# lxd99/TPNet

Hardware: AMD Instinct MI355X
Metric: temporal edges/sec (proj-update + pairwise readout) (higher is better)
Workload: dtype f32; 1 GPU; C2: Wikipedia-shape d=128 B=1000, L=3, synthetic S(8227,1000,E,span) stream of 2399000 edges, decoder-level unit (2 readouts + update per edge); batch=1000, dim=128, num_layer=3, nodes=9228, parallelism=single GPU

## Files before the change

tpnet_amd/csrc/plan.hip:

```cpp
#include "wplan_common.hpp"
#include "arena.hpp"
#include "sort_tmp.hpp"

#include <cstdlib>
#include <cstring>
#include <rocprim/block/block_radix_sort.hpp>
#include <rocprim/device/device_radix_sort.hpp>
#include <rocprim/device/device_segmented_radix_sort.hpp>
#include <rocprim/iterator/counting_iterator.hpp>
#include <rocprim/iterator/transform_iterator.hpp>

#ifdef TPNET_STAMPS
#define PSTAMP(slot)                                                                          \
    do {                                                                                      \
        if (dbg && blockIdx.x == 0 && threadIdx.x == 0) {                                     \
            dbg[(slot) * 2 + 0] = __builtin_amdgcn_s_memtime();                               \
            dbg[(slot) * 2 + 1] = __builtin_amdgcn_s_memrealtime();                           \
        }                                                                                     \
    } while (0)
#else
#define PSTAMP(slot) do { } while (0)
#endif

namespace tpnet {
// ... 606 lines not shown
    while (K < Kmax && (int64_t)K * K < (int64_t)num * nb) ++K;
    const int64_t nw0 = (nb + K - 1) / K;
    return (int)((nb + nw0 - 1) / nw0);
}

WPlanner choose_wplanner(const tpnet_state& st, const WPlan* p, int64_t Ec, int64_t batch, int K, uint32_t flags) {
    static const int no3 = TPNET_DEV_INT(NO_PLAN3, 0);
    static const int max3 = TPNET_DEV_INT(PLAN3_MAX_BATCHES, 1 << 30);
    const bool small = batch <= PLAN_ONE_MAX;
    if (!(flags & (TPNET_FLAG_PLAN_SORTED | TPNET_FLAG_PLAN_HASHED)) &&
        (p ? wplan_dense_applies(st, *p, Ec, batch, K) : small && wplan_dense_eligible(st.N, st.d, st.L, batch)))
        return {wplan_dense_build, wplan_dense_writeback, true, 256};
    if (!(flags & TPNET_FLAG_PLAN_SORTED) &&
        (p ? !no3 && (Ec + batch - 1) / batch <= max3 && wplan3_applies(st, Ec, batch, K) : small))
        return {wplan3_build, wplan3_writeback, true, WIN_MAX_WINDOWS};
    return {wplan_build, launch_wwriteback, false, 0};
}

bool wplan_medium_chains(int d) {
    static const int off = TPNET_DEV_INT(NO_MEDIUM, 0);
    if (off || d % 4 != 0) return false;
    const Geom g = pick_geom(d);
    return g.w == 4 && d == g.lpp * g.vpl * 4;
}

uint32_t wplan_heavy_threshold(int K, int64_t batch, int d) {
    static const int env = TPNET_DEV_INT(WIN_HEAVY, 0);
    if (env > 0) return (uint32_t)env;
    if (wplan_medium_chains(d)) return 128u;
    const int64_t t = (int64_t)K * batch * d / 24576;
    return (uint32_t)(t < 16 ? 16 : (t > 96 ? 96 : t));
}

int64_t wplan_max_chunk_edges(int64_t batch, int d, int L) {
    static const char* env = TPNET_DEV_STR(WIN_CHUNK_MB);
    const int64_t log_cap = (env ? (int64_t)atoi(env) : 16384) << 20;
    int64_t e = log_cap / (2 * (int64_t)L * d * 4);
    const int64_t hard = (int64_t)(WREF_SLOT_MASK >> 1);
    if (e > hard) e = hard;
    if (e > 65535 * batch) e = 65535 * batch;
    e = e / batch * batch;
    return e < batch ? batch : e;
}

static void wplan_layout(Arena& a, WPlan& p, int64_t Ec, int64_t batch, int64_t N, int d, int L, bool own_log) {
    const size_t nc = 2 * (size_t)Ec;
    const size_t nw = (size_t)((Ec + batch - 1) / batch);
    plan_layout(a, p.base, Ec, batch);
    a.skip(256);
    p.wscr = a.take<uint32_t>(3 * align256(nc * 4) / 4);
    a.skip(nc * 2);
    p.wdesc = a.take<WinDesc>(nw);
    a.skip(256);
    p.e_ref = a.take<uint32_t>(3 * (size_t)Ec);
    p.e_g = a.take<float>(3 * (size_t)Ec);
    p.log = own_log ? a.take<float>(nc * (size_t)L * (size_t)d) : nullptr;
    p.node_lo = a.take<uint32_t>((size_t)N);
    p.node_hi = a.take<uint32_t>((size_t)N);
    p.inv = a.take<uint32_t>(nc);
    p.rhead = a.take<uint32_t>(nc);
    const size_t zero0 = a.off;
    p.wmask = a.take<unsigned long long>((size_t)N);
    p.wcls = a.take<uint32_t>(2 * WIN_MAX_WINDOWS * 8 + WIN_MAX_WINDOWS);
    p.wzero_bytes = a.off - zero0;
    p.wtab = a.take<char>(wplan3_table_bytes(Ec, batch));
    p.wblk = (uint32_t*)a.take<char>(wplan3_blk_bytes(Ec, batch));
// ... 245 lines not shown
            const uint32_t c8 = ch.cnt > 255u ? 255u : ch.cnt;
            lk[j] = chain_head ? (((uint32_t)w << 8) | (255u - c8)) : lk_none;
            if (chain_head) p.chains_sparse[j] = ch;
        }
    }
}

__global__ void k_gather_chains(WPlan p, const uint32_t* __restrict__ lk, const uint32_t* __restrict__ lv, int64_t nc,
                                int64_t nw, uint32_t heavy_threshold, uint32_t lk_none) {
    if (blockIdx.x == gridDim.x - 1) {
        auto lb = [&](uint32_t key) {
            int64_t lo = 0, hi = nc;
            while (lo < hi) {
                const int64_t mid = (lo + hi) >> 1;
                if (lk[mid] < key) lo = mid + 1; else hi = mid;
            }
            return lo;
        };
        const uint32_t thr8 = heavy_threshold > 254u ? 254u : heavy_threshold;
        for (int64_t w = threadIdx.x; w < nw; w += blockDim.x) {
            const int64_t a = lb((uint32_t)w << 8);
            const int64_t h = lb(((uint32_t)w << 8) | (255u - thr8));
            const int64_t z = lb((uint32_t)(w + 1) << 8);
            WinDesc D;
            D.start = (uint32_t)a;
            D.n_heavy = (uint32_t)(h - a);
            D.n_chains = (uint32_t)(z - a);
            D.n_ext = D.n_heavy;
            D.n_ext1 = D.n_heavy;
            {
                const int64_t m = lb(((uint32_t)w << 8) | (255u - (WIN_MED_MIN - 1u)));
                D.n_med = (uint32_t)((m > h ? m : h) - a);
            }
            D.pad1 = D.pad2 = 0;
            p.wdesc[w] = D;
        }
        return;
    }
    for (int64_t i = (int64_t)blockIdx.x * blockDim.x + threadIdx.x; i < nc; i += (int64_t)(gridDim.x - 1) * blockDim.x) {
        if (lk[i] >= lk_none) continue;
        p.chains[i] = p.chains_sparse[lv[i]];
    }
}

template <typename K>
__device__ __forceinline__ void edge_refs(uint32_t bx, uint32_t nbx, WPlan p, const K* __restrict__ keys, const int64_t* __restrict__ src,
                            const int64_t* __restrict__ dst, const int64_t* __restrict__ neg, int64_t Ec, int64_t B,
                            int64_t N, int batch_bits, double lambda, const NodeMeta* __restrict__ meta) {
    const int nwhich = neg ? 3 : 2;
    const int64_t tot = (int64_t)nwhich * Ec;
    const int64_t nc = 2 * Ec;
    for (int64_t x = (int64_t)bx * blockDim.x + threadIdx.x; x < tot; x += (int64_t)nbx * blockDim.x) {
        const int which = (int)(x / Ec);
        const int64_t e = x - (int64_t)which * Ec;
        int64_t node = which == 0 ? src[e] : (which == 1 ? dst[e] : neg[e]);
        if ((uint64_t)node >= (uint64_t)N) node = 0;
        const int64_t b = e / B;
        uint32_t ref;
        float g;
        bool done = false;
        if (which < 2) {
            const int64_t e0b = b * B;
            const int64_t neb = (Ec - e0b < B) ? (Ec - e0b) : B;
            const uint32_t orig = (uint32_t)(2 * e0b + (which ? neb : 0) + (e - e0b));
            done = version_before_own_run<K>(p, keys, batch_bits, node, b, p.inv[orig], p.base.desc, meta, lambda,
                                             p.base.desc[b].now, ref, g);
        }
// ... 82 lines not shown
```

tpnet_amd/csrc/tpnet_common.h:

```cpp
#pragma once
#include <hip/hip_runtime.h>
#include <stdint.h>
#include <stdlib.h>
#include <initializer_list>
#include <new>
#include "../../include/tpnet_hip.h"
#include "tpnet_dev.h"
#include "event_set.hpp"

#ifdef TPNET_DEV
static inline int tpnet_dev_env_int(const char* name, int dflt) { const char* v = getenv(name); return v ? atoi(v) : dflt; }
#define TPNET_DEV_INT(NAME, DFLT) tpnet_dev_env_int("TPNET_DEV_" #NAME, (DFLT))
#define TPNET_DEV_STR(NAME) getenv("TPNET_DEV_" #NAME)
#else
#define TPNET_DEV_INT(NAME, DFLT) (DFLT)
#define TPNET_DEV_STR(NAME) ((const char*)nullptr)
#endif

namespace tpnet {

struct NodeMeta {
    uint32_t ver;
    uint32_t pad0;
    double tref[2];
// ... 203 lines not shown
               int64_t Ec, int64_t batch, double now_time, const double* t_prev_dev, double lambda, uint32_t flags,
               hipStream_t s);

static constexpr uint32_t ROLE_READOUT = 1u << 16;
static constexpr uint32_t ROLE_UPDATE = 1u << 17;
static constexpr uint32_t STEP_FUSE = 1u << 18;
static constexpr uint32_t STEP_ITEMS_FIRST = 1u << 20;
static constexpr uint32_t STEP_HAS_POS = 1u << 21;
static constexpr uint32_t STEP_HAS_NEG = 1u << 22;
static constexpr uint32_t PLAN_FUSE = 1u << 19;

static constexpr int WIN_MAX_BATCHES = 64;
static constexpr uint32_t WREF_TABLE = 1u << 31;
static constexpr uint32_t WREF_RUN_HEAD = 1u << 30;
static constexpr uint32_t WREF_RUN_TAIL = 1u << 29;
static constexpr uint32_t WREF_BLK_HEAD = 1u << 28;
static constexpr uint32_t WREF_BLK_TAIL = 1u << 27;
static constexpr uint32_t WREF_LAST_RUN = 1u << 26;
static constexpr uint32_t WREF_SLOT_MASK = (1u << 26) - 1;
static constexpr int WIN_MAX_WINDOWS = 64;
static constexpr int WIN_BLOCK = 8;

static constexpr uint32_t WIN_MED_MIN = 16;
__host__ __device__ inline int wchain_med_classes(uint32_t thr) {
    const int c = (32 - __builtin_clz(thr | 1u)) - 4;
    return c < 0 ? 0 : (c > 6 ? 6 : c);
}
__host__ __device__ inline int wchain_class(uint32_t cnt, uint32_t thr) {
    if (cnt > thr) return 0;
    const int dl = (32 - __builtin_clz(thr | 1u)) - (32 - __builtin_clz(cnt | 1u));
    return 1 + (dl > 6 ? 6 : (dl < 0 ? 0 : dl));
}

struct WinDesc {
    uint32_t start;
    uint32_t n_heavy;
    uint32_t n_chains;
    uint32_t n_ext;
    uint32_t n_ext1;
    uint32_t n_med;
    uint32_t pad1, pad2;
};

struct Chain {
    uint32_t j0;
    uint32_t cnt;
    int32_t target;
    uint32_t prev_ref;
    float g_first;
    uint32_t pad0, pad1, pad2;
};
static_assert(sizeof(Chain) == 32, "Chain must be 32 bytes");

struct WRec {
    int32_t partner;
    float coef;
    uint32_t ref;
    float g;
    float dec;
    int32_t target;
    uint32_t bc;
    uint32_t spare;
};
static_assert(sizeof(WRec) == 32, "WRec must be 32 bytes");

struct WPlan {
    Plan base;
    WRec* rec;
    uint32_t* wscr;
    WinDesc* wdesc;
    Chain* chains;
    Chain* chains_sparse;
    uint32_t* lk_in;
    uint32_t* lk_out;
    uint32_t* lv_in;
// ... 28 lines not shown
    const int64_t *src, *dst, *neg;
    const double* t;
    int64_t Ec, batch;
    double now_time;
    const double* t_prev_dev;
    double lambda;
    bool want_readout;
    bool replay;
    int64_t own = -1;
    uint32_t* status = nullptr;
};
int wplan_build(const tpnet_state& st, const WPlan& p, const WPlanArgs& a, hipStream_t s);
int wplan3_build(const tpnet_state& st, const WPlan& p, const WPlanArgs& a, hipStream_t s);
int wplan_dense_build(const tpnet_state& st, const WPlan& p, const WPlanArgs& a, hipStream_t s);
int launch_wwriteback(const tpnet_state& st, const WPlan& p, int64_t Ec, int64_t batch, uint32_t launch_id, hipStream_t s, int64_t own = -1);
int wplan3_writeback(const tpnet_state& st, const WPlan& p, int64_t Ec, int64_t batch, uint32_t launch_id, hipStream_t s, int64_t own = -1);
int wplan_dense_writeback(const tpnet_state& st, const WPlan& p, int64_t Ec, int64_t batch, uint32_t launch_id, hipStream_t s, int64_t own = -1);
bool wplan3_applies(const tpnet_state& st, int64_t Ec, int64_t batch, int K);
size_t wplan3_table_bytes(int64_t Ec, int64_t batch);
size_t wplan3_blk_bytes(int64_t Ec, int64_t batch);
bool wplan_dense_eligible(int64_t N, int d, int L, int64_t batch);
size_t wplan_dense_bytes(int64_t Ec, int64_t batch, int64_t N, int d, int L);
bool wplan_dense_applies(const tpnet_state& st, const WPlan& p, int64_t Ec, int64_t batch, int K);
bool wplan_dense_applies_shard(const tpnet_state& st, const WPlan& p, int64_t Ec, int64_t batch, int K);

struct WPlanner {
    decltype(&wplan_build) build;
    decltype(&launch_wwriteback) writeback;
    bool replayable;
    int max_windows;
};
WPlanner choose_wplanner(const tpnet_state& st, const WPlan* p, int64_t Ec, int64_t batch, int K, uint32_t flags);
uint32_t wplan_heavy_threshold(int K, int64_t batch, int d);
bool wplan_medium_chains(int d);
int launch_wstep(const tpnet_state& st, const StreamArgs& a, const WPlan& p, int64_t j, int64_t Ec, int64_t batch,
                 double lambda, uint32_t flags, hipStream_t s);
int check_state(const tpnet_state* st);

static inline bool aligned16(std::initializer_list<const void*> ps) {
    uintptr_t a = 0;
    for (const void* p : ps) a |= reinterpret_cast<uintptr_t>(p);
    return (a & 15) == 0;
}

extern thread_local int g_last_hip_error;
#define TPNET_HIP_TRY(expr)                                   \
    do {                                                      \
        hipError_t _e = (expr);                               \
        if (_e != hipSuccess) {                               \
            tpnet::g_last_hip_error = (int)_e;                \
            return TPNET_ERR_HIP;                             \
        }                                                     \
    } while (0)
#define TPNET_CATCH_BAD_ALLOC \
    catch (const std::bad_alloc&) { tpnet::g_last_hip_error = (int)hipErrorOutOfMemory; return TPNET_ERR_HIP; }

}
```

tpnet_amd/csrc/wplan3.hip:

```cpp
#include "wplan_common.hpp"

namespace tpnet {

size_t wplan3_table_bytes(int64_t Ec, int64_t batch) {
    const size_t nb = (size_t)((Ec + batch - 1) / batch);
    return wplan3_h2_bytes(Ec) + 256 + nb * wplan3_seg(batch) * sizeof(HEnt) + 256;
}
size_t wplan3_blk_bytes(int64_t Ec, int64_t batch) {
    const size_t nblk = (size_t)((Ec + batch - 1) / batch) * wplan3_bpb(batch);
    return 2 * nblk * 9 * sizeof(uint32_t) + 256;
}

template <int BS, int IPT>
__global__ __launch_bounds__(BS) void k_wsort(WTmp q, BatchDesc* __restrict__ desc, const int64_t* __restrict__ src_c,
                                              const int64_t* __restrict__ dst_c, const double* __restrict__ t_c, int64_t Ec,
                                              int32_t Bfull, int64_t N, int node_bits, double now_time,
                                              const double* __restrict__ t_prev, double lambda, int L, uint32_t* err, int KW) {
    __shared__ WSortShared<BS, IPT> sh;
    wsort_batch<BS, IPT, false>(sh, q, desc, src_c, dst_c, t_c, Ec, Bfull, N, node_bits, now_time, t_prev, lambda, L, err, KW,
                                (int64_t)blockIdx.x, nullptr);
}


__global__ __launch_bounds__(256) void k_wchains(WPlan p, WTmp q, int64_t Ec, int64_t Bfull, int64_t nb, uint32_t bpb) {
// ... 188 lines not shown
                                           int64_t w, int64_t e0b, double Tb, double Tnow, double lambda,
                                           const NodeMeta* __restrict__ meta, const uint32_t* cabs, int want_edges,
                                           const OwnSide me, const OwnSide other) {
    const uint32_t f = me.base + me.sb + me.ri;
    VRef pr = other.ver;
    if ((uint32_t)me.partner != other.node)
        pr = version_before_batch(p, q, Bfull, (int64_t)me.partner, b, meta);
    uint32_t out = (me.fl & WT_STRUCT_MASK) | pr.ref;
    float dec = 1.0f;
    if (me.fl & WREF_RUN_HEAD) {
        if (me.fl & WT_CHAIN_HEAD) {
            float g_first = 1.0f;
            if (me.ver.ref & WREF_TABLE) g_first = decay3_f32(lambda, Tb - me.ver.t_src);
            else dec = decay3_f32(lambda, Tb - me.ver.t_src);
            const int c = wchain_class(me.cnt, p.heavy_thr);
            const int64_t blk = b * q.bpb + (me.x - 2 * e0b) / 256;
            uint4* rec = reinterpret_cast<uint4*>(p.chains + (cabs[w * WCLS + c] + q.blkbase[blk * 9 + c] + me.aux));
            rec[0] = make_uint4(f, me.cnt, me.node, me.ver.ref);
            rec[1] = make_uint4(__float_as_uint(g_first), 0u, 0u, 0u);
        } else {
            dec = decay3_f32(lambda, Tb - me.ver.t_src);
        }
    }
    if ((me.fl & WT_WIN_LAST) && (w >= 63 || (me.wm >> (unsigned)(w + 1)) == 0ull)) out |= WREF_LAST_RUN;
    wrec_store(p.rec, f, me.partner, me.coef, out, decay3_f32(lambda, Tb - pr.t_src), dec, (int32_t)me.node, (uint32_t)b);
    if (want_edges) {
        p.e_ref[(int64_t)sd * Ec + e] = me.ver.ref;
        p.e_g[(int64_t)sd * Ec + e] = decay3_f32(lambda, Tnow - me.ver.t_src);
    }
}

__global__ __launch_bounds__(256) void k_wrefs(WPlan p, WTmp q, const int64_t* __restrict__ neg, int64_t Ec, int64_t Bfull,
                                               int64_t nb, int64_t N, double lambda, const NodeMeta* __restrict__ meta,
                                               uint32_t fgrid, int want_edges) {
    const int KW = p.K;
    const BatchDesc* __restrict__ desc = p.base.desc;
    if (blockIdx.x >= fgrid) {
        for (int64_t e = (int64_t)(blockIdx.x - fgrid) * blockDim.x + threadIdx.x; e < Ec;
             e += (int64_t)(gridDim.x - fgrid) * blockDim.x) {
            int64_t node = neg[e];
            if ((uint64_t)node >= (uint64_t)N) node = 0;
            const int64_t b = e / Bfull;
            const VRef r = version_before_batch(p, q, Bfull, node, b, meta);
            p.e_ref[2 * Ec + e] = r.ref;
            p.e_g[2 * Ec + e] = decay3_f32(lambda, desc[b].now - r.t_src);
        }
        return;
    }
    __shared__ uint32_t cabs[WIN_MAX_WINDOWS * WCLS];
    const int64_t nw = (nb + KW - 1) / KW;
    if (threadIdx.x < 64) {
        const int wv = threadIdx.x;
        uint32_t n = 0, t8[WCLS];
#pragma unroll
        for (int k = 0; k < WCLS; ++k) {
            t8[k] = wv < nw ? q.wtot[wv * 9 + k] : 0u;
            n += t8[k];
        }
        uint32_t at = wave_incl_scan(n) - n;
        if (blockIdx.x == 0 && wv < nw) {
            WinDesc D;
            D.start = at;
            D.n_heavy = t8[0];
            D.n_chains = n;
            D.n_ext = t8[0] + t8[1] + t8[2];
            D.n_ext1 = t8[0] + t8[1];
            D.n_med = 0;
            for (int k = 0; k <= wchain_med_classes(p.heavy_thr); ++k) D.n_med += t8[k];
            D.pad1 = D.pad2 = 0;
            p.wdesc[wv] = D;
        }
#pragma unroll
        for (int k = 0; k < WCLS; ++k) {
            cabs[wv * WCLS + k] = at;
            at += t8[k];
        }
    }
    __syncthreads();
    for (int64_t e = (int64_t)blockIdx.x * blockDim.x + threadIdx.x; e < Ec; e += (int64_t)fgrid * blockDim.x) {
        const int64_t b = e / Bfull;
        const int64_t w = b / KW;
        const int64_t e0b = b * Bfull;
        const int64_t neb = (Ec - e0b < Bfull) ? (Ec - e0b) : Bfull;
        const double Tb = desc[b].t_last, Tnow = desc[b].now;
        const int64_t x0 = q.binv[2 * e0b + (e - e0b)], x1 = q.binv[2 * e0b + neb + (e - e0b)];
        OwnSide s0, s1;
        side_load(q, x0, s0);
        side_load(q, x1, s1);
        const CEnt* c0 = cfind(q, s0.node, (uint32_t)w);
        const CEnt* c1 = cfind(q, s1.node, (uint32_t)w);
        s0.wm = p.wmask[s0.node];
        s1.wm = p.wmask[s1.node];
        side_version(p, q, Bfull, w, c0, meta, s0);
        side_version(p, q, Bfull, w, c1, meta, s1);
        side_store(p, q, Bfull, Ec, e, 0, b, w, e0b, Tb, Tnow, lambda, meta, cabs, want_edges, s0, s1);
        side_store(p, q, Bfull, Ec, e, 1, b, w, e0b, Tb, Tnow, lambda, meta, cabs, want_edges, s1, s0);
    }
}

static WTmp wtmp_full(const tpnet_state& st, const WPlan& p, int64_t Ec, int64_t batch) {
    const int64_t nb = (Ec + batch - 1) / batch;
    WTmp q = wtmp_of(p, (size_t)(2 * Ec));
// ... 36 lines not shown
    const WTmp q = wtmp_full(st, p, Ec, batch);
    int64_t grid = (st.N + 7) / 8;
    if (grid > 16384) grid = 16384;
    hipLaunchKernelGGL(k_wwriteback_nodes, dim3((unsigned)grid), dim3(256), 0, s, st, p, q, batch, launch_id);
    TPNET_HIP_TRY(hipGetLastError());
    return TPNET_OK;
}

bool wplan3_applies(const tpnet_state& st, int64_t Ec, int64_t batch, int K) {
    if (K < 1 || batch < 1 || batch > PLAN_ONE_MAX) return false;
    const int64_t nb = (Ec + batch - 1) / batch;
    const int64_t nw = (nb + K - 1) / K;
    int node_bits = 1;
    while (node_bits < 63 && (1ll << node_bits) < st.N) ++node_bits;
    return nw <= WIN_MAX_WINDOWS && nb < 65536 && node_bits <= 31 && (int64_t)K * batch * 2 < (1 << 24) &&
           2 * Ec < (int64_t)WREF_SLOT_MASK;
}

int wplan3_build(const tpnet_state& st, const WPlan& p, const WPlanArgs& a, hipStream_t s) {
    const int64_t *src = a.src, *dst = a.dst, *neg = a.neg, Ec = a.Ec, batch = a.batch;
    const double *t = a.t, *t_prev_dev = a.t_prev_dev, now_time = a.now_time, lambda = a.lambda;
    const bool want_readout = a.want_readout, replay = a.replay;
    if (!wplan3_applies(st, Ec, batch, p.K) || !p.wmask || !p.wcls || !p.wtab || !p.wblk) return TPNET_ERR_BAD_ARG;
    const int64_t nb = (Ec + batch - 1) / batch;
    WTmp q = wtmp_full(st, p, Ec, batch);
    const int64_t nw = (nb + p.K - 1) / p.K;
    int node_bits = 1;
    while (node_bits < 31 && (1ll << node_bits) < st.N) ++node_bits;
    const NodeMeta* meta = reinterpret_cast<const NodeMeta*>(st.meta);
    const int nwhich = want_readout ? (neg ? 3 : 2) : 0;
    const int ngrid = (nwhich == 3) ? ((int)((Ec + 255) / 256) > 2048 ? 2048 : (int)((Ec + 255) / 256)) : 0;
    if (replay) {
        if (ngrid) {
            hipLaunchKernelGGL(k_wrefs, dim3(ngrid), dim3(256), 0, s, p, q, neg, Ec, batch, nb, st.N, lambda, meta, 0u, 0);
            TPNET_HIP_TRY(hipGetLastError());
        }
        return TPNET_OK;
    }
    const size_t h2_used = (q.direct2 ? (size_t)nw * (size_t)st.N : (size_t)q.hcap) * sizeof(CEnt);
    TPNET_HIP_TRY(hipMemsetAsync(p.wmask, 0, p.wzero_bytes + h2_used, s));
    {
#define TPNET_WSORT(BS_, IPT_)                                                                                              \
    hipLaunchKernelGGL((k_wsort<BS_, IPT_>), dim3((unsigned)nb), dim3(BS_), 0, s, q, p.base.desc, src, dst, t, Ec,           \
                       (int32_t)batch, st.N, node_bits, now_time, t_prev_dev, lambda, (int)st.L, st.err, (int)p.K)
        const int64_t n2 = 2 * batch;
        TPNET_FOR_BATCH_TILE(n2, TPNET_WSORT);
#undef TPNET_WSORT
        TPNET_HIP_TRY(hipGetLastError());
    }
    hipLaunchKernelGGL(k_wchains, dim3((unsigned)(nb * q.bpb)), dim3(256), 0, s, p, q, Ec, batch, nb, q.bpb);
    hipLaunchKernelGGL(k_wscan, dim3((unsigned)((nb + p.K - 1) / p.K)), dim3(9 * 64), 0, s, p, q, nb);
    TPNET_HIP_TRY(hipGetLastError());
    int egrid = (int)((Ec + 255) / 256);
    if (egrid > 8192) egrid = 8192;
    hipLaunchKernelGGL(k_wrefs, dim3(egrid + ngrid), dim3(256), 0, s, p, q, neg, Ec, batch, nb, st.N, lambda, meta,
                       (uint32_t)egrid, nwhich >= 2 ? 1 : 0);
    TPNET_HIP_TRY(hipGetLastError());
    return TPNET_OK;
}

}
```

tpnet_amd/csrc/wplan_dense.hip:

```cpp
#include "wplan_dense.hpp"

namespace tpnet {

static constexpr int64_t DENSE_SHARD_MAX_BATCH = 8192;
bool wplan_dense_eligible(int64_t N, int d, int L, int64_t batch) {
    static const int off = TPNET_DEV_INT(NO_PLAN_DENSE, 0);
    if (off || batch < 1 || batch > DENSE_SHARD_MAX_BATCH || N > (int64_t)DENSE_MAX_CHUNKS * 256) return false;
    return (int64_t)N * 12 <= batch * (int64_t)L * d * 4;
}

size_t wplan_dense_bytes(int64_t Ec, int64_t batch, int64_t N, int d, int L) {
    if (!wplan_dense_eligible(N, d, L, batch)) return 0;
    return measured([&](Arena& a) { DView v; dense_layout(a, v, Ec, batch, N); });
}

struct DArgs {
    const int64_t* src;
    const int64_t* dst;
    const int64_t* neg;
    const double* t;
    const double* t_prev;
    const NodeMeta* meta;
    uint32_t* err;
    int64_t Ec, Bfull, N, nb, nw;
// ... 396 lines not shown
    for (int64_t b0 = bw0; b0 < bw1; b0 += UB) {
        uint32_t l[UB];
#pragma unroll
        for (int k = 0; k < UB; ++k) {
            const int64_t b = (b0 + k < bw1) ? b0 + k : bw1 - 1;
            l[k] = (uint32_t)D.len[b * D.Ns + nld];
        }
#pragma unroll
        for (int k = 0; k < UB; ++k) {
            const int64_t b = b0 + k;
            if (b < bw1) {
                if (live) D.m[b * D.Ns + n] = make_uint2(run, l[k] | (prevb << 16));
                run += l[k];
                prevb = l[k] ? (uint32_t)b : prevb;
            }
        }
    }
    __syncthreads();
    if (tid < 8) {
        uint32_t before = 0;
        for (int k = 0; k < DCH / 8; ++k) before += part[k * 8 + tid];
        D.cpre[(size_t)c * npair + w * 8 + tid] = before;
        if (c == a.nchunks - 1) D.ptot[w * 8 + tid] = before + D.ccnt[(size_t)c * npair + w * 8 + tid];
    }
    if (w == a.nw - 1) {
        if (!live) run = 0;
        uint32_t total;
        const uint32_t ex = block_excl_scan<DCH>(run, wsum, total);
        if (live) { D.tot[n] = run; D.lastb[n] = prevb; D.base[n] = ex; }
        if (tid == 0) D.ctot[c] = total;
    }
}

__global__ __launch_bounds__(DCH) void k_dense_place(WPlan p, WTmp q, DView D, DArgs a) {
    __shared__ uint32_t wsum[DCH / 64];
    __shared__ uint32_t cbase[DENSE_MAX_CHUNKS];
    __shared__ uint32_t lstart[DENSE_MAX_WINDOWS * 8];
    __shared__ double tlast[DENSE_TL];
    const int tid = threadIdx.x;
    const int npair = (int)a.nw * 8;
    const double* tl = a.nb <= DENSE_TL ? tlast : nullptr;
    if (tl)
        for (int64_t b = tid; b < a.nb; b += DCH) tlast[b] = p.base.desc[b].t_last;
    {
        uint32_t carry = 0;
        for (int64_t c0 = 0; c0 < a.nchunks; c0 += DCH) {
            const int64_t c = c0 + tid;
            const uint32_t v = c < a.nchunks ? D.ctot[c] : 0u;
            uint32_t tot;
            const uint32_t ex = block_excl_scan<DCH>(v, wsum, tot);
            if (c < a.nchunks) cbase[c] = carry + ex;
            carry += tot;
        }
        carry = 0;
        for (int i0 = 0; i0 < npair; i0 += DCH) {
            const int i = i0 + tid;
            const uint32_t v = i < npair ? D.ptot[i] : 0u;
            uint32_t tot;
            const uint32_t ex = block_excl_scan<DCH>(v, wsum, tot);
            if (i < npair) lstart[i] = carry + ex;
            carry += tot;
        }
        __syncthreads();
    }
    if (blockIdx.x == 0) {
        for (int64_t w = tid; w < a.nw; w += DCH) {
            uint32_t t8[8], n = 0;
#pragma unroll
            for (int k = 0; k < 8; ++k) { t8[k] = D.ptot[w * 8 + k]; n += t8[k]; }
            WinDesc W;
            W.start = lstart[w * 8];
            W.n_heavy = t8[0];
            W.n_chains = n;
            W.n_ext = t8[0] + t8[1] + t8[2];
            W.n_ext1 = t8[0] + t8[1];
            W.n_med = 0;
            for (int k = 0; k <= wchain_med_classes(p.heavy_thr); ++k) W.n_med += t8[k];
            W.pad1 = W.pad2 = 0;
            p.wdesc[w] = W;
        }
    }
    const int64_t gid = (int64_t)blockIdx.x * DCH + tid, gsz = (int64_t)gridDim.x * DCH;
    for (int64_t n = gid; n < a.N; n += gsz) D.basef[n] = D.base[n] + cbase[n / DCH];
    const int64_t nc = 2 * a.Ec;
    const bool shard = a.own < a.N;
    const int64_t n_neg = a.nwhich == 3 ? a.Ec : 0;
    const int64_t items = nc + n_neg + ((shard && a.nwhich >= 2) ? a.Ec : 0);
    for (int64_t x = gid; x < items; x += gsz) {
        if (x < nc) {
            if (shard) {
                const int64_t b = x / (2 * a.Bfull);
                if (x - 2 * b * a.Bfull >= (int64_t)p.base.desc[b].n_light) continue;
            }
            dense_place(p, q, D, a, lstart, cbase, tl, x);
        } else if (x < nc + n_neg) {
            dense_neg_c(p, D, a, cbase, tl, x - nc);
        } else {
            dense_neg_c(p, D, a, cbase, tl, x - nc - n_neg, 1);
        }
    }
}

__global__ __launch_bounds__(256) void k_wplan_dense_negs(WPlan p, DView D, DArgs a) {
    for (int64_t e = (int64_t)blockIdx.x * blockDim.x + threadIdx.x; e < a.Ec; e += (int64_t)gridDim.x * blockDim.x)
        dense_neg(p, D, a, D.basef, e);
}

__global__ __launch_bounds__(256) void k_wwriteback_dense(tpnet_state S, WPlan p, DView D, uint32_t bid, int64_t own) {
    constexpr int LANES = 32;
    const int per = S.L * S.d;
    const int pv = per / 4;
// ... 39 lines not shown
    DArgs a;
    a.src = pa.src; a.dst = pa.dst; a.neg = pa.neg; a.t = pa.t; a.t_prev = pa.t_prev_dev;
    a.meta = reinterpret_cast<const NodeMeta*>(st.meta);
    a.err = st.err;
    a.Ec = Ec; a.Bfull = batch; a.N = st.N; a.nb = nb; a.nw = (nb + p.K - 1) / p.K;
    a.now_time = pa.now_time; a.lambda = pa.lambda;
    int node_bits = 1;
    while (node_bits < 31 && (1ll << node_bits) < st.N) ++node_bits;
    a.node_bits = node_bits;
    a.L = st.L;
    a.nwhich = pa.want_readout ? (pa.neg ? 3 : 2) : 0;
    a.nchunks = (int32_t)((st.N + DCH - 1) / DCH);
    a.own = own;
    a.status = pa.status;
    if (replay) {
        if (a.nwhich == 3) {
            hipLaunchKernelGGL(k_wplan_dense_negs, dim3(grid_1d(Ec, 2048)), dim3(256), 0, s, p, D, a);
            TPNET_HIP_TRY(hipGetLastError());
        }
        return TPNET_OK;
    }
#define TPNET_WDENSE(BS_, IPT_) hipLaunchKernelGGL((k_dense_sort<BS_, IPT_>), dim3((unsigned)nb), dim3(BS_), 0, s, p, q, D, a)
    const int64_t n2 = 2 * batch;
    static const int no_group = TPNET_DEV_INT(DENSE_SORT, 0);
    if (shard) hipLaunchKernelGGL((k_dense_sort_shard<1024, 4>), dim3((unsigned)nb), dim3(1024), 0, s, p, q, D, a);
    else if (!no_group && n2 <= 2048 && st.N <= DENSE_GROUP_MAX_N)
        hipLaunchKernelGGL((k_dense_group<1024, 2, DENSE_GROUP_MAX_N>), dim3((unsigned)nb), dim3(1024), 0, s, p, q, D, a);
    else TPNET_FOR_BATCH_TILE(n2, TPNET_WDENSE);
#undef TPNET_WDENSE
    const unsigned bgrid = (unsigned)((int64_t)a.nchunks * a.nw);
    hipLaunchKernelGGL(k_dense_win, dim3(bgrid), dim3(DCH), 0, s, p, D, a);
    hipLaunchKernelGGL(k_dense_pre, dim3(bgrid), dim3(DCH), 0, s, p, D, a);
    static_assert(DCH == 256, "grid_1d counts workgroups of 256");
    hipLaunchKernelGGL(k_dense_place, dim3(grid_1d(3 * Ec, 4096)), dim3(DCH), 0, s, p, q, D, a);
    TPNET_HIP_TRY(hipGetLastError());
    return TPNET_OK;
}

int wplan_dense_writeback(const tpnet_state& st, const WPlan& p, int64_t Ec, int64_t batch, uint32_t launch_id, hipStream_t s,
                          int64_t own) {
    if ((st.L * st.d) % 4 != 0) return TPNET_ERR_BAD_ARG;
    if (own < 0 || own > st.N) own = st.N;
    const DView D = dview_of(p, Ec, batch, st.N);
    int64_t grid = (own + 7) / 8;
    if (grid > 16384) grid = 16384;
    if (grid < 1) grid = 1;
    hipLaunchKernelGGL(k_wwriteback_dense, dim3((unsigned)grid), dim3(256), 0, s, st, p, D, launch_id, own);
    TPNET_HIP_TRY(hipGetLastError());
    return TPNET_OK;
}

}
```

tpnet_amd/csrc/wstep.hip:

```cpp
#include "readout.hpp"
#include "wplan_common.hpp"

namespace tpnet {

static constexpr int WB = 256;
#ifndef TPNET_WPIPE_MINW
#define TPNET_WPIPE_MINW 4
#endif
constexpr int wpipe_min_waves(int lpp, int vpl, int l, bool full) {
    return (lpp <= 32 && vpl == 1) ? TPNET_WPIPE_MINW
         : (lpp == 32 && vpl == 2) ? ((full && l <= 3) ? 3 : 2)
         : (lpp == 64 && vpl == 1) ? (full ? 3 : 2)
         : 2;
}

__device__ __forceinline__ float pow_rep(float g, int n) {
    float r = 1.0f;
    for (int z = 0; z < n; ++z) r *= g;
    return r;
}

__device__ __forceinline__ const float* partner_row(const tpnet_state& S, const WPlan& P, int layer, int32_t pv,
                                                    uint32_t ref, float g, float& gp) {
    const int d = S.d, L = S.L;
    if (layer == 1) {
        gp = 1.0f;
        return S.p0 + (int64_t)pv * d;
    }
    gp = pow_rep(g, layer - 1);
    if (ref & WREF_TABLE) return S.q + (((int64_t)(ref & 1u) * S.N + pv) * L + (layer - 2)) * (int64_t)d;
    return P.log + ((int64_t)(ref & WREF_SLOT_MASK) * L + (layer - 2)) * (int64_t)d;
}

__device__ __forceinline__ const float* chain_start(const tpnet_state& S, const WPlan& P, const Chain& c, int layer,
                                                    float& g0) {
    const int d = S.d, L = S.L;
    g0 = pow_rep(c.g_first, layer);
    if (c.prev_ref & WREF_TABLE)
        return S.q + (((int64_t)(c.prev_ref & 1u) * S.N + c.target) * L + (layer - 1)) * (int64_t)d;
    return P.log + ((int64_t)(c.prev_ref & WREF_SLOT_MASK) * L + (layer - 1)) * (int64_t)d;
}

template <int LPP, int VPL, bool FULL>
__device__ __forceinline__ void chain_light(const tpnet_state& S, const WPlan& P, Chain c, bool valid, int layer,
                                            double lambda, int gl, unsigned long long* dbg) {
    (void)dbg;
    STAMP(5);
    constexpr int W = 4, F = VPL * W, U = (F == 4) ? 8 : 4;
    const int d = S.d, L = S.L;
    const int nvec = d / W;
    if (!valid) { c.cnt = 0; c.target = 0; c.j0 = 0; c.prev_ref = WREF_TABLE; c.g_first = 1.0f; }
    float g0;
    const float* qold = chain_start(S, P, c, layer, g0);
    const bool from_table = (c.prev_ref & WREF_TABLE) != 0;
    const WRec* __restrict__ rec = P.rec;

    for (int c0 = 0; c0 < (FULL ? 1 : nvec); c0 += LPP * VPL) {
        float acc[F], sblk[F], srun[F];
#pragma unroll
        for (int j = 0; j < VPL; ++j) {
            const int vi = c0 + j * LPP + gl;
            ldv_maybe<W, FULL>(qold, vi, valid && vi < nvec, &acc[j * W]);
        }
#pragma unroll
        for (int x = 0; x < F; ++x) { sblk[x] = 0.0f; srun[x] = 0.0f; }
        bool firstblk = false;
        float cur_dec = 1.0f;
        int32_t nx_pv = 0;
        float nx_w = 0.0f, nx_glog = 1.0f, nx_decr = 1.0f;
        uint32_t nx_ref = 0u;
        auto fetch_meta = [&](uint32_t r0) {
            const uint32_t jm = c.j0 + r0 + (uint32_t)gl;
            const bool mine = r0 + (uint32_t)gl < c.cnt;
            const WRecWalk rw = wrec_load_walk(rec, mine ? jm : c.j0);
            const WRecEnds re = wrec_load_ends(rec, mine ? jm : c.j0);
            nx_pv = mine ? rw.partner : 0;
            nx_w = mine ? rw.coef : 0.0f;
            nx_ref = mine ? rw.ref : 0u;
            nx_glog = mine ? rw.g : 1.0f;
            nx_decr = mine ? re.dec : 1.0f;
        };
        fetch_meta(0u);
        for (uint32_t r0 = 0; __any(r0 < c.cnt); r0 += LPP) {
            const int32_t my_pv = nx_pv;
            const float my_w = nx_w;
            const uint32_t my_ref = nx_ref;
            const float my_glog = nx_glog;
            const float my_dec = pow_rep(nx_decr, layer);
            if (__any(r0 + LPP < c.cnt)) fetch_meta(r0 + LPP);
            float my_gp;
            const float* my_row = partner_row(S, P, layer, my_pv, my_ref, my_glog, my_gp);
            const uint32_t n_here = (r0 < c.cnt) ? ((c.cnt - r0 < (uint32_t)LPP) ? c.cnt - r0 : (uint32_t)LPP) : 0u;
            constexpr int US = U / 2;
            float rA[US][F], rB[US][F];
            auto issue = [&](uint32_t k0, float (&r)[US][F]) {
#pragma unroll
                for (int k = 0; k < US; ++k) {
                    const int sl = (int)k0 + k;
                    const bool ok = (uint32_t)sl < n_here;
                    const float* rp = reinterpret_cast<const float*>(__shfl((long long)reinterpret_cast<uintptr_t>(my_row), sl, LPP));
                    if (!ok) rp = S.p0;
#pragma unroll
                    for (int j = 0; j < VPL; ++j) {
                        const int vi = c0 + j * LPP + gl;
                        ldv_maybe<W, FULL>(rp, vi, ok && vi < nvec, &r[k][j * W]);
                    }
                }
            };
            auto consume = [&](uint32_t k0, const float (&r)[US][F]) {
#pragma unroll
                for (int k = 0; k < US; ++k) {
                    const int sl = (int)k0 + k;
                    if ((uint32_t)sl < n_here) {
                        const float w = __shfl(my_w, sl, LPP);
                        const float gp = __shfl(my_gp, sl, LPP);
                        const float dc = __shfl(my_dec, sl, LPP);
                        const uint32_t fl = (uint32_t)__shfl((int)my_ref, sl, LPP);
                        const uint32_t pos = c.j0 + r0 + k0 + (uint32_t)k;
                        const bool bh = (fl & WREF_BLK_HEAD) != 0;
#pragma unroll
                        for (int x = 0; x < F; ++x) {
                            const float m = (r[k][x] * gp) * w;
// ... 651 lines not shown
        BEND();
        return;
    }
    const WinDesc wd = P.wdesc[w];
    unsigned long long* dbg = (st.dbg_layer == layer) ? P.base.dbg : nullptr;
    (void)dbg;
    if (sidx < L) {
#ifdef TPNET_DEV
        if (st.dbg_skip & 1) return;
#endif
        const Chain* __restrict__ heavy = P.chains + wd.start;
        const uint32_t units = hub_chains(st, wd) * (uint32_t)st.CP;
        for (uint32_t h = rb; h < units; h += nblk)
            chain_heavy<LPH>(S, P, heavy[h / (uint32_t)st.CP], (int)(h % (uint32_t)st.CP), layer, lambda,
                             (uint32_t)(w * P.K), lds_u, dbg);
        BEND();
        return;
    }
    if (sidx < SL) {
        if constexpr (FULL) {
            const uint32_t n_hub = hub_chains(st, wd);
            const uint32_t n_big = big_chains(st, wd, n_hub);
            const Chain* __restrict__ list = P.chains + wd.start;
            for (uint32_t m = n_hub + rb; m < n_big; m += nblk) chain_medium<LPP, VPL, LWORDS>(S, P, list[m], layer, lds_u);
        }
        BEND();
        return;
    }
#ifdef TPNET_DEV
    if (st.dbg_skip & 2) return;
#endif
    const uint32_t n_hub = big_chains(st, wd, hub_chains(st, wd));
    const Chain* __restrict__ small = P.chains + wd.start + n_hub;
    const int64_t n_small = (int64_t)wd.n_chains - (int64_t)n_hub;
    for (int64_t base = (int64_t)rb * GPB; base < n_small; base += (int64_t)nblk * GPB) {
        const int64_t idx = base + g;
        const bool valid = idx < n_small;
        const Chain c = small[valid ? idx : 0];
        chain_light<LPP, VPL, FULL>(S, P, c, valid, layer, lambda, gl, dbg);
    }
    BEND();
}

static constexpr int WBS = 256;
__global__ __launch_bounds__(WB) void k_wwriteback(tpnet_state S, WPlan P, int64_t nc, uint32_t bid) {
    const int per = S.L * S.d;
    NodeMeta* meta = reinterpret_cast<NodeMeta*>(S.meta);
    __shared__ uint32_t n_list;
    __shared__ uint32_t l_pos[WBS];
    __shared__ int32_t l_node[WBS];
    __shared__ int32_t l_copy[WBS];
    for (int64_t j0 = (int64_t)blockIdx.x * WBS; j0 < nc; j0 += (int64_t)gridDim.x * WBS) {
        __syncthreads();
        if (threadIdx.x == 0) n_list = 0;
        __syncthreads();
        const int64_t j = j0 + threadIdx.x;
        if (threadIdx.x < WBS && j < nc && (wrec_load_walk(P.rec, (size_t)j).ref & WREF_LAST_RUN)) {
            const int32_t u = wrec_load_ends(P.rec, (size_t)j).target;
            const int c = (int)(meta[u].ver & 1u);
            const uint32_t k = atomicAdd(&n_list, 1u);
            l_pos[k] = (uint32_t)j;
            l_node[k] = u;
            l_copy[k] = c;
        }
        __syncthreads();
        const uint32_t n = n_list;
        if ((per & 3) == 0) {
            const uint32_t pv = (uint32_t)per / 4;
            const uint32_t tot = n * pv;
            for (uint32_t x0 = threadIdx.x; x0 < tot; x0 += 4 * WB) {
                const uint32_t xa = x0, xb = x0 + WB, xc = x0 + 2 * WB, xd = x0 + 3 * WB;
                const uint32_t ka = xa / pv, kb = (xb < tot ? xb : xa) / pv, kc = (xc < tot ? xc : xa) / pv, kd = (xd < tot ? xd : xa) / pv;
// ... 138 lines not shown
```

Baseline: 365.4 million edges/s.

## Process short chains with narrower 16-lane groups in a single-pass light path

Adds an n_wide count per window, so chains whose size class falls below a threshold (up to 8 or 16 records) are split off from the wide light path. Those short chains are processed by 16-lane groups with VPL=2 and a single-iteration loop that skips the prefetch of further metadata. More chains fit per workgroup and fewer lanes idle on short chains. This adds a new WinDesc field, threshold logic tied to K and the heavy threshold, and a template variant gated on RS.

After: 381.6 million edges/s (median of 6 runs). +4.4%, better.

```diff
diff --git a/tpnet_amd/csrc/plan.hip b/tpnet_amd/csrc/plan.hip
--- a/tpnet_amd/csrc/plan.hip
+++ b/tpnet_amd/csrc/plan.hip
@@ -662,6 +662,13 @@
     return (uint32_t)(t < 16 ? 16 : (t > 96 ? 96 : t));
 }
 
+uint32_t wplan_narrow_from(uint32_t thr, int K) {
+    static const int mode = TPNET_DEV_INT(WIN_NARROW, -1);
+    if (mode == 0 || mode > 2) return 8u;
+    const bool upto7 = mode < 0 ? K >= 14 : mode == 1;
+    return (uint32_t)wchain_short_from(thr, upto7 ? 3 : 2);
+}
+
 int64_t wplan_max_chunk_edges(int64_t batch, int d, int L) {
     static const char* env = TPNET_DEV_STR(WIN_CHUNK_MB);
     const int64_t log_cap = (env ? (int64_t)atoi(env) : 16384) << 20;
@@ -973,7 +980,8 @@
                 const int64_t m = lb(((uint32_t)w << 8) | (255u - (WIN_MED_MIN - 1u)));
                 D.n_med = (uint32_t)((m > h ? m : h) - a);
             }
-            D.pad1 = D.pad2 = 0;
+            D.n_wide = D.n_chains;
+            D.pad2 = 0;
             p.wdesc[w] = D;
         }
         return;
diff --git a/tpnet_amd/csrc/tpnet_common.h b/tpnet_amd/csrc/tpnet_common.h
--- a/tpnet_amd/csrc/tpnet_common.h
+++ b/tpnet_amd/csrc/tpnet_common.h
@@ -259,6 +259,11 @@
     return 1 + (dl > 6 ? 6 : (dl < 0 ? 0 : dl));
 }
 
+__host__ __device__ inline int wchain_short_from(uint32_t thr, int bits) {
+    const int k = (32 - __builtin_clz(thr | 1u)) - bits + 1;
+    return k < 1 ? 1 : (k > 7 ? 8 : k);
+}
+
 struct WinDesc {
     uint32_t start;
     uint32_t n_heavy;
@@ -266,8 +271,10 @@
     uint32_t n_ext;
     uint32_t n_ext1;
     uint32_t n_med;
-    uint32_t pad1, pad2;
-};
+    uint32_t n_wide;
+    uint32_t pad2;
+};
+static_assert(sizeof(WinDesc) == 32, "WinDesc must be 32 bytes");
 
 struct Chain {
     uint32_t j0;
@@ -362,6 +369,7 @@
 };
 WPlanner choose_wplanner(const tpnet_state& st, const WPlan* p, int64_t Ec, int64_t batch, int K, uint32_t flags);
 uint32_t wplan_heavy_threshold(int K, int64_t batch, int d);
+uint32_t wplan_narrow_from(uint32_t thr, int K);
 bool wplan_medium_chains(int d);
 int launch_wstep(const tpnet_state& st, const StreamArgs& a, const WPlan& p, int64_t j, int64_t Ec, int64_t batch,
                  double lambda, uint32_t flags, hipStream_t s);
diff --git a/tpnet_amd/csrc/wplan3.hip b/tpnet_amd/csrc/wplan3.hip
--- a/tpnet_amd/csrc/wplan3.hip
+++ b/tpnet_amd/csrc/wplan3.hip
@@ -244,7 +244,7 @@
 
 __global__ __launch_bounds__(256) void k_wrefs(WPlan p, WTmp q, const int64_t* __restrict__ neg, int64_t Ec, int64_t Bfull,
                                                int64_t nb, int64_t N, double lambda, const NodeMeta* __restrict__ meta,
-                                               uint32_t fgrid, int want_edges) {
+                                               uint32_t fgrid, int want_edges, uint32_t narrow_from) {
     const int KW = p.K;
     const BatchDesc* __restrict__ desc = p.base.desc;
     if (blockIdx.x >= fgrid) {
@@ -279,7 +279,9 @@
             D.n_ext1 = t8[0] + t8[1];
             D.n_med = 0;
             for (int k = 0; k <= wchain_med_classes(p.heavy_thr); ++k) D.n_med += t8[k];
-            D.pad1 = D.pad2 = 0;
+            D.n_wide = 0;
+            for (int k = 0; k < WCLS; ++k) D.n_wide += (uint32_t)k < narrow_from ? t8[k] : 0u;
+            D.pad2 = 0;
             p.wdesc[wv] = D;
         }
 #pragma unroll
@@ -382,7 +384,7 @@
     const int ngrid = (nwhich == 3) ? ((int)((Ec + 255) / 256) > 2048 ? 2048 : (int)((Ec + 255) / 256)) : 0;
     if (replay) {
         if (ngrid) {
-            hipLaunchKernelGGL(k_wrefs, dim3(ngrid), dim3(256), 0, s, p, q, neg, Ec, batch, nb, st.N, lambda, meta, 0u, 0);
+            hipLaunchKernelGGL(k_wrefs, dim3(ngrid), dim3(256), 0, s, p, q, neg, Ec, batch, nb, st.N, lambda, meta, 0u, 0, 8u);
             TPNET_HIP_TRY(hipGetLastError());
         }
         return TPNET_OK;
@@ -404,7 +406,7 @@
     int egrid = (int)((Ec + 255) / 256);
     if (egrid > 8192) egrid = 8192;
     hipLaunchKernelGGL(k_wrefs, dim3(egrid + ngrid), dim3(256), 0, s, p, q, neg, Ec, batch, nb, st.N, lambda, meta,
-                       (uint32_t)egrid, nwhich >= 2 ? 1 : 0);
+                       (uint32_t)egrid, nwhich >= 2 ? 1 : 0, wplan_narrow_from(p.heavy_thr, p.K));
     TPNET_HIP_TRY(hipGetLastError());
     return TPNET_OK;
 }
diff --git a/tpnet_amd/csrc/wplan_dense.hip b/tpnet_amd/csrc/wplan_dense.hip
--- a/tpnet_amd/csrc/wplan_dense.hip
+++ b/tpnet_amd/csrc/wplan_dense.hip
@@ -452,7 +452,7 @@
     }
 }
 
-__global__ __launch_bounds__(DCH) void k_dense_place(WPlan p, WTmp q, DView D, DArgs a) {
+__global__ __launch_bounds__(DCH) void k_dense_place(WPlan p, WTmp q, DView D, DArgs a, uint32_t narrow_from) {
     __shared__ uint32_t wsum[DCH / 64];
     __shared__ uint32_t cbase[DENSE_MAX_CHUNKS];
     __shared__ uint32_t lstart[DENSE_MAX_WINDOWS * 8];
@@ -496,7 +496,9 @@
             W.n_ext1 = t8[0] + t8[1];
             W.n_med = 0;
             for (int k = 0; k <= wchain_med_classes(p.heavy_thr); ++k) W.n_med += t8[k];
-            W.pad1 = W.pad2 = 0;
+            W.n_wide = 0;
+            for (int k = 0; k < 8; ++k) W.n_wide += (uint32_t)k < narrow_from ? t8[k] : 0u;
+            W.pad2 = 0;
             p.wdesc[w] = W;
         }
     }
@@ -602,7 +604,7 @@
     hipLaunchKernelGGL(k_dense_win, dim3(bgrid), dim3(DCH), 0, s, p, D, a);
     hipLaunchKernelGGL(k_dense_pre, dim3(bgrid), dim3(DCH), 0, s, p, D, a);
     static_assert(DCH == 256, "grid_1d counts workgroups of 256");
-    hipLaunchKernelGGL(k_dense_place, dim3(grid_1d(3 * Ec, 4096)), dim3(DCH), 0, s, p, q, D, a);
+    hipLaunchKernelGGL(k_dense_place, dim3(grid_1d(3 * Ec, 4096)), dim3(DCH), 0, s, p, q, D, a, wplan_narrow_from(p.heavy_thr, p.K));
     TPNET_HIP_TRY(hipGetLastError());
     return TPNET_OK;
 }
diff --git a/tpnet_amd/csrc/wstep.hip b/tpnet_amd/csrc/wstep.hip
--- a/tpnet_amd/csrc/wstep.hip
+++ b/tpnet_amd/csrc/wstep.hip
@@ -41,7 +41,7 @@
     return P.log + ((int64_t)(c.prev_ref & WREF_SLOT_MASK) * L + (layer - 1)) * (int64_t)d;
 }
 
-template <int LPP, int VPL, bool FULL>
+template <int LPP, int VPL, bool FULL, bool ONE = false>
 __device__ __forceinline__ void chain_light(const tpnet_state& S, const WPlan& P, Chain c, bool valid, int layer,
                                             double lambda, int gl, unsigned long long* dbg) {
     (void)dbg;
@@ -81,13 +81,13 @@
             nx_decr = mine ? re.dec : 1.0f;
         };
         fetch_meta(0u);
-        for (uint32_t r0 = 0; __any(r0 < c.cnt); r0 += LPP) {
+        for (uint32_t r0 = 0; ONE ? r0 == 0u : __any(r0 < c.cnt); r0 += LPP) {
             const int32_t my_pv = nx_pv;
             const float my_w = nx_w;
             const uint32_t my_ref = nx_ref;
             const float my_glog = nx_glog;
             const float my_dec = pow_rep(nx_decr, layer);
-            if (__any(r0 + LPP < c.cnt)) fetch_meta(r0 + LPP);
+            if (!ONE && __any(r0 + LPP < c.cnt)) fetch_meta(r0 + LPP);
             float my_gp;
             const float* my_row = partner_row(S, P, layer, my_pv, my_ref, my_glog, my_gp);
             const uint32_t n_here = (r0 < c.cnt) ? ((c.cnt - r0 < (uint32_t)LPP) ? c.cnt - r0 : (uint32_t)LPP) : 0u;
@@ -805,12 +805,27 @@
 #endif
     const uint32_t n_hub = big_chains(st, wd, hub_chains(st, wd));
     const Chain* __restrict__ small = P.chains + wd.start + n_hub;
-    const int64_t n_small = (int64_t)wd.n_chains - (int64_t)n_hub;
+    uint32_t n_wide = wd.n_chains;
+    if constexpr (RS) n_wide = wd.n_wide < n_hub ? n_hub : (wd.n_wide < wd.n_chains ? wd.n_wide : wd.n_chains);
+    const int64_t n_small = (int64_t)n_wide - (int64_t)n_hub;
     for (int64_t base = (int64_t)rb * GPB; base < n_small; base += (int64_t)nblk * GPB) {
         const int64_t idx = base + g;
         const bool valid = idx < n_small;
         const Chain c = small[valid ? idx : 0];
         chain_light<LPP, VPL, FULL>(S, P, c, valid, layer, lambda, gl, dbg);
+    }
+    if constexpr (RS) {
+        constexpr int NLPP = 16, NGPB = WB / NLPP;
+        const int ngl = threadIdx.x % NLPP;
+        const int ng = threadIdx.x / NLPP;
+        const Chain* __restrict__ shortc = small + n_small;
+        const int64_t n_short = (int64_t)wd.n_chains - (int64_t)n_hub - n_small;
+        for (int64_t base = (int64_t)rb * NGPB; base < n_short; base += (int64_t)nblk * NGPB) {
+            const int64_t idx = base + ng;
+            const bool valid = idx < n_short;
+            const Chain c = shortc[valid ? idx : 0];
+            chain_light<NLPP, 2, FULL, true>(S, P, c, valid, layer, lambda, ngl, dbg);
+        }
     }
     BEND();
 }
```
